# scalable-matrix/CRP-SpMM

Measured on AMD Instinct MI355X. Metric: SpMM GFLOP/s (pwtk stand-in n=256, fp64), higher is better.
Workload: dtype f64

## Files before the change

### crp-spmm_amd/_lib.py

```python
import ctypes as C
import os

_HERE = os.path.dirname(os.path.abspath(__file__))
LIB_PATH = os.environ.get("CRPSPMM_LIB_PATH") or os.path.join(_HERE, "lib", "libcrpspmm_hip.so")


class CrpLibraryError(RuntimeError):
    pass


class CrpHipError(RuntimeError):
    pass


c_int_p = C.POINTER(C.c_int)
c_dbl_p = C.POINTER(C.c_double)
c_ll_p = C.POINTER(C.c_longlong)
c_sz_p = C.POINTER(C.c_size_t)
c_u64_p = C.POINTER(C.c_uint64)

A2A_FN = C.CFUNCTYPE(None, C.c_void_p, c_int_p, c_int_p, C.c_int)
A2AV_FN = C.CFUNCTYPE(None, C.c_void_p, c_int_p, c_int_p, c_int_p, c_int_p, c_int_p, c_int_p)
AGV_FN = C.CFUNCTYPE(None, C.c_void_p, C.c_void_p, C.c_size_t, C.c_void_p, c_sz_p, c_sz_p)
BARRIER_FN = C.CFUNCTYPE(None, C.c_void_p)
# ... 45 lines not shown


class CrpspmmView(C.Structure):
    _fields_ = [(k, C.c_int) for k in ("np_glb", "rank_glb", "np_row", "np_col", "rank_row", "rank_col", "glb_m", "glb_n",
                                       "glb_k", "loc_A_srow", "loc_A_erow", "loc_A_nrow", "loc_A_nnz", "loc_A_nnz_s",
                                       "rd_B_srow", "rd_B_erow", "loc_B_scol", "loc_B_ecol", "loc_B_ncol", "loc_B_srow",
                                       "loc_B_erow", "loc_B_nrow", "a2a_B_finegrain")] + \
               [("loc_A_rowptr", c_int_p), ("loc_A_colidx", c_int_p), ("loc_A_val", c_dbl_p), ("red_B", c_dbl_p),
                ("loc_C", c_dbl_p), ("n_exec", C.c_int)] + \
               [(k, C.c_double) for k in ("t_init", "t_exec", "t_rd_A", "t_agv_A", "t_rd_B", "t_a2a_B", "t_spmm", "t_rd_C",
                                          "t_exec_nr")] + \
               [(k, C.c_size_t) for k in ("nelem_A_rd", "nelem_A_agv", "nelem_B_rd", "nelem_B_a2av", "nelem_B_a2av_min")]


_V = C.c_void_p
_I = C.c_int
_LL = C.c_longlong

SIGNATURES = {
    "crp_hip_version": (C.c_char_p, []),
    "crp_hip_device_count": (_I, [c_int_p]),
    "crp_hip_set_device": (_I, [_I]),
    "crp_hip_get_device": (_I, [c_int_p]),
    "crp_hip_device_info": (_I, [_I, C.c_char_p, c_int_p, c_sz_p]),
    "crp_hip_device_bus_id": (_I, [C.c_char_p, C.c_size_t]),
    "crp_dev_malloc": (_I, [C.POINTER(_V), C.c_size_t]),
    "crp_dev_free": (_I, [_V]),
    "crp_dev_memset": (_I, [_V, _I, C.c_size_t, _V]),
    "crp_dev_memcpy": (_I, [_V, _V, C.c_size_t, _I, _V]),
    "crp_dev_memcpy2d": (_I, [_V, C.c_size_t, _V, C.c_size_t, C.c_size_t, C.c_size_t, _I, _V]),
    "crp_host_malloc": (_I, [C.POINTER(_V), C.c_size_t]),
    "crp_host_free": (_I, [_V]),
    "crp_dev_ptr_is_device": (_I, [_V, c_int_p]),
    "crp_stream_create": (_I, [C.POINTER(_V)]),
    "crp_stream_destroy": (_I, [_V]),
    "crp_stream_sync": (_I, [_V]),
    "crp_event_create": (_I, [C.POINTER(_V)]),
    "crp_event_destroy": (_I, [_V]),
    "crp_event_record": (_I, [_V, _V]),
    "crp_event_sync": (_I, [_V]),
    "crp_stream_wait_event": (_I, [_V, _V]),
    "crp_event_elapsed_ms": (_I, [_V, _V, C.POINTER(C.c_float)]),
    "crp_csr_dev_create": (_I, [_I, _I, c_int_p, c_int_p, c_dbl_p, C.POINTER(_V)]),
    "crp_csr_dev_create_dv": (_I, [_I, _I, c_int_p, c_int_p, c_dbl_p, _V, c_int_p, C.POINTER(_V)]),
    "crp_csr_dev_destroy": (_I, [C.POINTER(_V)]),
    "crp_csr_dev_update_values": (_I, [_V, _V, _V]),
    "crp_csr_dev_set_rowmap": (_I, [_V, c_int_p, _I]),
    "crp_csr_dev_nrow": (_I, [_V]),
    "crp_csr_dev_nnz": (_LL, [_V]),
    "crp_csr_dev_bytes": (_LL, [_V]),
    "crp_csr_dev_row_part_comm_size": (_I, [_V, _I, c_int_p, c_int_p, c_int_p, c_int_p]),
    "crp_csr_dev_auto_variant": (_I, [_V]),
    "crp_csr_dev_reordered": (_I, [_V]),
    "crp_csr_dev_resolved_variant": (_I, [_V, _I]),
    "crp_csr_dev_last_variant": (_I, [_V]),
    "crp_csr_dev_lattice": (_I, [_V]),
    "crp_csr_dev_team2_compact": (_I, [_V]),
    "crp_panel_format_host": (_I, [_I, c_int_p, c_int_p, c_dbl_p, _I, c_int_p, C.POINTER(c_int_p), C.POINTER(c_int_p),
                                   C.POINTER(C.POINTER(C.c_uint)), C.POINTER(c_dbl_p), C.POINTER(_LL),
                                   C.POINTER(c_int_p), c_int_p]),
    "crp_team_format_host": (_I, [_I, c_int_p, c_int_p, c_dbl_p, c_int_p, c_int_p, C.POINTER(c_int_p), C.POINTER(c_int_p),
                                  C.POINTER(c_int_p), C.POINTER(C.POINTER(C.c_uint)), C.POINTER(c_int_p)]),
    "crp_probe_copy": (_I, [C.c_longlong, _V, _V, _I, _V, _V]),
    "crp_probe_stamp": (_I, [_V, _V]),
    "crp_stream_create_cu_mask": (_I, [C.POINTER(_V), _I, C.POINTER(C.c_uint)]),
    "crp_team2_format_host_grid": (_I, [C.POINTER(c_int_p), c_int_p]),
# ... 171 lines not shown
```

### crp-spmm_amd/csrc/dispatch.cpp

```cpp
#include "dispatch.h"
#include "locality.h"
#include "panel_format.h"

namespace crp {

constexpr int TEAM2_MIN_N = 96;
constexpr int TEAM2_HALF_FULL_LO = 61, TEAM2_HALF_FULL_HI = 64;
constexpr int TEAM2_MIN_N_NOLATTICE = 48;
constexpr int TEAM2_MIN_N_DENSE = 33;
constexpr int TEAM2_MIN_N_SPARSE = 33;
constexpr int TEAM2_MIN_N_F32 = 32, TEAM2_MIN_N_F32_SPARSE = 65;

FormatOrder format_order(int nrow, int ncol, const int *rowptr, const int *colidx, bool two_source)
{
    FormatOrder o;
    const long long nnz = rowptr[nrow];
    if (!(nnz > 0 && nrow >= 2048 && nrow == ncol && !two_source && nnz <= 200000000LL))
        return o;
    const int mode = knobs().reorder;
    std::vector<int> perm;
    if (mode == 0 || !locality_reorder(nrow, ncol, rowptr, colidx, 8, &perm)) return o;
    o.f_rowptr.assign((size_t) nrow + 1, 0);
    for (int i = 0; i < nrow; i++) o.f_rowptr[(size_t) i + 1] = o.f_rowptr[(size_t) i] + (rowptr[perm[(size_t) i] + 1] - rowptr[perm[(size_t) i]]);
    o.f_colidx.resize((size_t) nnz);
    o.f_nz.resize((size_t) nnz);
    for (int i = 0; i < nrow; i++)
    {
        const int r = perm[(size_t) i];
        int q = o.f_rowptr[(size_t) i];
        for (int pz = rowptr[r]; pz < rowptr[r + 1]; pz++, q++)
        {
            o.f_colidx[(size_t) q] = colidx[pz];
// ... 56 lines not shown
}
template bool team2_applicable<double>(const Operand &);
template bool team2_applicable<float>(const Operand &);

static bool team2_width(const MatrixTraits &t, int n)
{
    return n >= t.team2_min_n || (t.team2_min_n == TEAM2_MIN_N && n >= TEAM2_HALF_FULL_LO && n <= TEAM2_HALF_FULL_HI);
}

int resolve_f64(const MatrixTraits &t, const Operand &op, int variant, bool team2r_refused, const Knobs &k)
{
    const int n = op.n;
    const bool rows = t.nnz > 0 && t.nrow >= 8;
    int v = (variant == 0) ? t.auto_variant : variant;
    if (variant == 0 && t.team2_pays && team2_width(t, n) && team2_applicable<double>(op)) v = 5;
    const int panel_or_csr = panel_applicable(op) && t.nnz > 0 ? 3 : 1;
    if (v == 5) return team2_applicable<double>(op) && rows ? 5 : panel_or_csr;
    const int G = n <= 32 ? 4 : 2;
    const bool team2r_auto = k.team2r >= 0 ? k.team2r != 0 : (t.panels_sparse && !team2r_refused);
    if (variant == 0 && t.team2_pays && team2r_auto && n <= 64 && rows && team2r_applicable(op, G)) v = team2r_refused ? 3 : 7;
    if (v == 7) return team2r_applicable(op, G) && rows ? 7 : panel_or_csr;
    if (v >= 2 && (!panel_applicable(op) || t.nnz == 0)) v = 1;
    return v;
}

int resolve_f32(const MatrixTraits &t, const Operand &op, int variant)
{
    const int min_n = t.panels_sparse ? TEAM2_MIN_N_F32_SPARSE : TEAM2_MIN_N_F32;
    const bool team = (variant == 5 || (variant == 0 && t.team2_pays && op.n >= min_n)) && t.nnz > 0 && t.nrow >= 8 &&
                      team2_applicable<float>(op);
    return team ? 5 : 1;
}

bool team2_compact(double fill, bool for_f32)
{
    return knobs().team2_compact >= 0 ? knobs().team2_compact != 0 : (fill < 0.4 || !for_f32);
}

}
```

### crp-spmm_amd/csrc/dispatch.h

```cpp
#pragma once
#include <stdint.h>
#include <vector>
#include "knobs.h"

namespace crp {

struct FormatOrder
{
    std::vector<int>      perm, f_rowptr, f_colidx;
    std::vector<uint32_t> f_nz;
};
FormatOrder format_order(int nrow, int ncol, const int *rowptr, const int *colidx, bool two_source);

struct MatrixTraits
{
    int       nrow = 0;
    long long nnz = 0;
    int       auto_variant = 1;
    bool      team2_pays = false;
    int       team2_min_n = 96;
    bool      panels_sparse = false;
};
MatrixTraits matrix_traits(int nrow, const int *rowptr, const int *colidx);

struct Operand
{
    int       n = 0;
    long long ldB0 = 0, ldB1 = 0, ldC = 0;
    bool      has_b1 = false;
    bool      aligned16 = true;
};
bool panel_applicable(const Operand &op);
bool team2r_applicable(const Operand &op, int G);
template <typename T> bool team2_applicable(const Operand &op);

int resolve_f64(const MatrixTraits &t, const Operand &op, int variant, bool team2r_refused, const Knobs &k);
int resolve_f32(const MatrixTraits &t, const Operand &op, int variant);

bool team2_compact(double fill, bool for_f32);

}
```

### crp-spmm_amd/csrc/hip_api.hip

```cpp
#include <hip/hip_runtime.h>
#include <stdio.h>
#include <stdlib.h>
#include <string.h>
#include <new>
#include <memory>
#include <algorithm>
#include <array>
#include <vector>
#include "crpspmm_hip.h"
#include "kernels.h"
#include "panel_format.h"
#include "dispatch.h"
#include "locality.h"
#include "knobs.h"

template <typename T> struct DevBuf
{
    T *p = nullptr;
    DevBuf() = default;
    DevBuf(DevBuf &&o) noexcept : p(o.p) { o.p = nullptr; }
    DevBuf &operator=(DevBuf &&o) noexcept { std::swap(p, o.p); return *this; }
    ~DevBuf() { reset(); }
    void reset() { if (p) (void) hipFree(p); p = nullptr; }
    hipError_t alloc(size_t bytes) { reset(); return hipMalloc((void **) &p, bytes); }
// ... 363 lines not shown
int crp_dev_memcpy(void *dst, const void *src, size_t bytes, int kind, void *stream)
{
    if (bytes == 0) return 0;
    if (kind < 0 || kind > 2) return -1;
    CRP_TRY(hipMemcpyAsync(dst, src, bytes, k_copy_kinds[kind], (hipStream_t) stream));
    return 0;
}

int crp_dev_memcpy2d(void *dst, size_t dpitch, const void *src, size_t spitch, size_t width_bytes, size_t height,
                     int kind, void *stream)
{
    if (width_bytes == 0 || height == 0) return 0;
    if (kind < 0 || kind > 2) return -1;
    CRP_TRY(hipMemcpy2DAsync(dst, dpitch, src, spitch, width_bytes, height, k_copy_kinds[kind], (hipStream_t) stream));
    return 0;
}

int crp_host_malloc(void **ptr, size_t bytes)
{
    if (ptr == NULL) return -1;
    *ptr = NULL;
    if (bytes == 0) return 0;
    CRP_TRY(hipHostMalloc(ptr, bytes, hipHostMallocDefault));
    return 0;
}

int crp_host_free(void *ptr)
{
    if (ptr == NULL) return 0;
    CRP_TRY(hipHostFree(ptr));
    return 0;
}

int crp_dev_ptr_is_device(const void *ptr, int *is_dev)
{
    if (is_dev == NULL) return -1;
    *is_dev = 0;
    if (ptr == NULL) return 0;
    hipPointerAttribute_t attr;
    hipError_t e = hipPointerGetAttributes(&attr, ptr);
    if (e != hipSuccess)
    {
        (void) hipGetLastError();
        return 0;
    }
    *is_dev = (attr.type == hipMemoryTypeDevice) ? 1 : 0;
    return 0;
}

int crp_stream_create(void **stream)
{
    if (stream == NULL) return -1;
    hipStream_t s;
    CRP_TRY(hipStreamCreateWithFlags(&s, hipStreamNonBlocking));
    *stream = (void *) s;
    return 0;
}
int crp_stream_create_cu_mask(void **stream, int nwords, const unsigned *mask32)
{
    if (stream == NULL || nwords <= 0 || mask32 == NULL) return -1;
    hipStream_t s;
    CRP_TRY(hipExtStreamCreateWithCUMask(&s, (uint32_t) nwords, mask32));
    *stream = (void *) s;
    return 0;
}
int crp_probe_copy(long long bytes, const void *src, void *dst, int blocks, unsigned long long *stamps, void *stream)
// ... 314 lines not shown
    if (C == NULL || (B0 == NULL && B1 == NULL && A->nnz > 0)) return -1;
    if (ldC < n || (B0 && ldB0 < n) || (B1 && ldB1 < n)) return -4;
    const hipStream_t s = (hipStream_t) stream;
    if (A->val32 == nullptr)
    {
        CRP_TRY(A->val32.alloc(sizeof(float) * (size_t) (A->nnz > 0 ? A->nnz : 1)));
        CRP_TRY(crp::convert_f64_f32(A->nnz, A->val, A->val32, s));
    }
    crp::SpmmArgsF32 a;
    a.nrow = A->nrow; a.n = n; a.rowptr = A->rowptr; a.colidx = A->colidx; a.val = A->val32;
    a.B0 = B0; a.ldB0 = ldB0; a.B1 = B1; a.ldB1 = ldB1; a.C = C; a.ldC = ldC; a.rowmap = A->rowmap;
    A->last_variant = crp::resolve_f32(A->traits, operand_of(n, B0, ldB0, B1, ldB1, C, ldC), variant);
    if (A->last_variant == 1) return (int) crp::spmm_rm_f32_rowgroup(a, s);
    const int rc = ensure_team2(A, s, true);
    if (rc != 0) return rc;
    Team2Dev &d = A->team2;
    if (d.tval32 == nullptr)
    {
        CRP_TRY(d.tval32.alloc(sizeof(float) * ((size_t) d.value_entries + 1024)));
        CRP_TRY(hipMemsetAsync(d.tval32, 0, sizeof(float) * ((size_t) d.value_entries + 1024), s));
        CRP_TRY(crp::convert_f64_f32(d.value_entries, d.tval, d.tval32, s));
    }
    if (A->rowmap_fmt != nullptr) a.rowmap = A->rowmap_fmt;
    crp::Team2Args t;
    team2_args(d, &t);
    return (int) crp::spmm_rm_f32_team2(t, a, s);
}

int crp_csr_dev_auto_variant(crp_csr_dev_p A) { return A ? A->traits.auto_variant : -1; }
int crp_csr_dev_reordered(crp_csr_dev_p A) { return A ? (A->ord.perm.empty() ? 0 : 1) : -1; }
int crp_csr_dev_resolved_variant(crp_csr_dev_p A, int n)
{
    return A ? crp::resolve_f64(A->traits, operand_of(n, nullptr, n, nullptr, 0, nullptr, n), 0, A->team2r_refused, crp::knobs()) : -1;
}
int crp_csr_dev_last_variant(crp_csr_dev_p A) { return A ? A->last_variant : -1; }
int crp_csr_dev_lattice(crp_csr_dev_p A) { return A ? ((A->team2.built && A->team2.lattice) ? 1 : 0) : -1; }
int crp_csr_dev_team2_compact(crp_csr_dev_p A) { return (A && A->team2.built) ? (A->team2.compact ? 1 : 0) : -1; }

int crp_panel_format_host(int nrow, const int *rowptr, const int *colidx, const double *val, int R, int *npanel,
                          int **pptr, int **pcol, unsigned **pmask4, double **pval, long long *real_entries,
                          int **porder, int *norder)
{
    if (nrow < 0 || rowptr == NULL || (R != 4 && R != 8) || !npanel || !pptr || !pcol || !pmask4 || !pval) return -1;
    crp::PanelHost h;
    crp::build_panels(nrow, rowptr, colidx, val, R, &h);
    *npanel = h.npanel;
    *pptr = dup(h.pptr);
    *pcol = dup(h.pcol);
    *pmask4 = dup(h.pmask4);
    *pval = dup(h.pval);
    if (real_entries) *real_entries = h.real_entries;
    if (norder) *norder = (int) h.porder.size();
    if (porder) *porder = dup(h.porder);
    return 0;
}

int crp_team_format_host(int nrow, const int *rowptr, const int *colidx, const double *val, int *nteam, int *lattice,
                         int **tpanel, int **tptr, int **tcol, unsigned **tmask, int **torder)
{
    if (nrow < 0 || rowptr == NULL || !nteam || !tpanel || !tptr || !tcol || !tmask || !torder) return -1;
    crp::PanelHost h;
    crp::build_panels(nrow, rowptr, colidx, val, 8, &h, false);
    crp::TeamHost th;
    crp::build_teams(h, nrow, rowptr, colidx, &th);
    *nteam = th.nteam;
    if (lattice) *lattice = th.lattice ? 1 : 0;
// ... 167 lines not shown
```

### crp-spmm_amd/csrc/kernels.h

```cpp
#pragma once
#include <hip/hip_runtime.h>
#include <stdint.h>

namespace crp {

struct SpmmArgs
{
    int nrow;
    int n;
    const int    *rowptr;
    const int    *colidx;
    const double *val;
    const double *B0;
    int64_t       ldB0;
    const double *B1;
    int64_t       ldB1;
    double       *C;
    int64_t       ldC;
    const int    *rowmap;
};

struct SpmmArgsF32
{
    int nrow;
// ... 48 lines not shown
    int G;
    int nteam;
    int ngrid;
    const int      *tgrid;
    const int      *tpanel;
    const int      *tinfo;
    const uint32_t *trec;
    const long long *tvoff;
    const double   *tval;
    uint32_t       *tent;
};

bool spmm_narrow_applicable(const PanelArgs &p, const SpmmArgs &a);
hipError_t spmm_rm_f64_narrow(const PanelArgs &p, const SpmmArgs &a, hipStream_t s);

hipError_t spmm_rm_f64_rowgroup(const SpmmArgs &a, hipStream_t s);
hipError_t spmm_cm_f64(const SpmmArgs &a, hipStream_t s);
hipError_t spmm_rm_f64_panel(const PanelArgs &p, const SpmmArgs &a, hipStream_t s);

hipError_t spmm_rm_f64_team2r(const Team2NArgs &t, const SpmmArgs &a, hipStream_t s);
hipError_t team2r_fill_rows(const Team2NArgs &t, const SpmmArgs &a, hipStream_t s);

hipError_t spmm_rm_f64_team2(const Team2Args &t, const SpmmArgs &a, hipStream_t s);
hipError_t spmm_rm_f32_team2(const Team2Args &t, const SpmmArgsF32 &a, hipStream_t s);

hipError_t spmm_rm_f32_rowgroup(const SpmmArgsF32 &a, hipStream_t s);

hipError_t gather_rows_f64(int layout, int nidx, int n, const int *ridx, const double *src, int64_t lds,
                           double *dst, int64_t ldd, hipStream_t s);
hipError_t scatter_rows_f64(int layout, int nidx, int n, const int *ridx, const double *src, int64_t lds,
                            double *dst, int64_t ldd, hipStream_t s);
hipError_t scatter_vals_f64(int64_t n, const uint32_t *map, const double *src, double *dst, hipStream_t s);
hipError_t convert_f64_f32(int64_t n, const double *src, float *dst, hipStream_t s);
hipError_t transpose_f64(int nrow, int ncol, const double *src, int64_t lds, double *dst, int64_t ldd,
                         hipStream_t s);
hipError_t gather_rows_f32(int layout, int nidx, int n, const int *ridx, const float *src, int64_t lds,
                           float *dst, int64_t ldd, hipStream_t s);
hipError_t scatter_rows_f32(int layout, int nidx, int n, const int *ridx, const float *src, int64_t lds,
                            float *dst, int64_t ldd, hipStream_t s);
hipError_t transpose_f32(int nrow, int ncol, const float *src, int64_t lds, float *dst, int64_t ldd, hipStream_t s);
hipError_t row_part_comm_size(int nrow, int ncol, const int *rowptr, const int *colidx, int nblk, const int *rblk_dev, const int *xd_dev,
                              unsigned *bits, int *comm_dev, int *bad_dev, hipStream_t s);
hipError_t probe_copy(int64_t bytes, const void *src, void *dst, int blocks, unsigned long long *stamps, hipStream_t s);
hipError_t probe_stamp(unsigned long long *out, hipStream_t s);

}
```

### crp-spmm_amd/csrc/knobs.cpp

```cpp
#include <stdlib.h>
#include <string.h>
#include <algorithm>
#include "knobs.h"

namespace crp {

static int env_int(const char *name, int dflt)
{
    const char *v = getenv(name);
    return (v != NULL && *v != 0) ? atoi(v) : dflt;
}

static bool env_is(const char *name, const char *what)
{
    const char *v = getenv(name);
    return v != NULL && strcmp(v, what) == 0;
}

static Knobs read_knobs()
{
    Knobs k;
    k.timing = env_int("CRPSPMM_TIMING", 0) != 0;
    k.num_threads = std::max(0, env_int("CRPSPMM_NUM_THREADS", env_int("OMP_NUM_THREADS", 0)));
    k.sync_release = getenv("CRPSPMM_SYNC_RELEASE") != NULL;
    k.spmm_variant = env_int("CRPSPMM_SPMM_VARIANT", 0);
    k.reorder = env_int("CRPSPMM_REORDER", -1);
    k.panel_order = env_int("CRPSPMM_PANEL_ORDER", -1);
    k.team2_compact = env_int("CRPSPMM_TEAM2_COMPACT", -1);
    k.team2r = env_int("CRPSPMM_TEAM2R", -1);
    k.t2_latorder = env_int("CRPSPMM_T2_LATORDER", 1) != 0;
    k.overlap = env_int("CRPSPMM_OVERLAP", 1);
    k.exchange_host = env_is("CRPSPMM_EXCHANGE", "host");
    k.replicate_host = env_is("CRPSPMM_REPLICATE", "host");
    {
        const char *v = getenv("CRPSPMM_RCCL_TIMEOUT");
        const double t = v ? atof(v) : 120.0;
        k.rccl_timeout = t > 0.0 ? t : 120.0;
    }
    k.rccl_blocking = env_int("CRPSPMM_RCCL_BLOCKING", 0) != 0;
    k.engine_a_static = env_int("CRPSPMM_ENGINE_A_STATIC", -1);
    return k;
}

const Knobs &knobs()
{
    static const bool live = env_int("CRPSPMM_KNOBS_LIVE", 0) != 0;
    static Knobs k = read_knobs();
    if (live) k = read_knobs();
    return k;
}

}
```

### crp-spmm_amd/csrc/knobs.h

```cpp
#pragma once

namespace crp {

struct Knobs
{
    bool   timing;
    int    num_threads;
    bool   sync_release;
    int    spmm_variant;
    int    reorder;
    int    panel_order;
    int    team2_compact;
    int    team2r;
    bool   t2_latorder;
    int    overlap;
    bool   exchange_host;
    bool   replicate_host;
    double rccl_timeout;
    bool   rccl_blocking;
    int    engine_a_static;
};

const Knobs &knobs();

}
```

### crp-spmm_amd/csrc/row_kernels.hip

```cpp
#include <hip/hip_runtime.h>
#include <algorithm>
#include <stdint.h>
#include "kernels.h"

namespace crp {

typedef double d2 __attribute__((ext_vector_type(2)));

static inline int grid_for(int64_t work)
{
    int64_t blocks = (work + 255) / 256;
    if (blocks > 2048) blocks = 2048;
    if (blocks < 1) blocks = 1;
    return (int) blocks;
}

template <int VW, bool GATHER>
__global__ __launch_bounds__(256) void move_rows_rm_kernel(
    const int64_t nidx, const int cpr , const int *__restrict__ ridx,
    const double *__restrict__ src, const int64_t lds, double *__restrict__ dst, const int64_t ldd)
{
    const int64_t total = nidx * (int64_t) cpr;
    for (int64_t t = (int64_t) blockIdx.x * 256 + threadIdx.x; t < total; t += (int64_t) gridDim.x * 256)
    {
// ... 224 lines not shown
{
    if (nrow <= 0 || ncol <= 0) return hipSuccess;
    dim3 grid((nrow + 31) / 32, (ncol + 31) / 32);
    hipLaunchKernelGGL(transpose_f32_kernel, grid, dim3(256), 0, s, nrow, ncol, src, lds, dst, ldd);
    return hipGetLastError();
}

__global__ __launch_bounds__(256) void scatter_vals_kernel(const int64_t n, const uint32_t *__restrict__ map,
                                                           const double *__restrict__ src, double *__restrict__ dst)
{
    for (int64_t i = (int64_t) blockIdx.x * 256 + threadIdx.x; i < n; i += (int64_t) gridDim.x * 256) dst[map[i]] = src[i];
}

hipError_t scatter_vals_f64(int64_t n, const uint32_t *map, const double *src, double *dst, hipStream_t s)
{
    if (n <= 0) return hipSuccess;
    hipLaunchKernelGGL(scatter_vals_kernel, dim3(grid_for(n)), dim3(256), 0, s, n, map, src, dst);
    return hipGetLastError();
}

__global__ void convert_f64_f32_kernel(const int64_t n, const double *__restrict__ src, float *__restrict__ dst)
{
    for (int64_t i = (int64_t) blockIdx.x * blockDim.x + threadIdx.x; i < n; i += (int64_t) gridDim.x * blockDim.x) dst[i] = (float) src[i];
}

hipError_t convert_f64_f32(int64_t n, const double *src, float *dst, hipStream_t s)
{
    if (n <= 0) return hipSuccess;
    const int blocks = (int) ((n + 255) / 256 < 4096 ? (n + 255) / 256 : 4096);
    hipLaunchKernelGGL(convert_f64_f32_kernel, dim3(blocks), dim3(256), 0, s, n, src, dst);
    return hipGetLastError();
}

__global__ __launch_bounds__(256) void probe_copy_kernel(const int64_t n16, const uint4 *__restrict__ src, uint4 *__restrict__ dst,
                                                          unsigned long long *__restrict__ stamps)
{
    if (threadIdx.x == 0) atomicMin(&stamps[0], (unsigned long long) wall_clock64());
    for (int64_t i = (int64_t) blockIdx.x * 256 + threadIdx.x; i < n16; i += (int64_t) gridDim.x * 256) dst[i] = src[i];
    __syncthreads();
    if (threadIdx.x == 0) atomicMax(&stamps[1], (unsigned long long) wall_clock64());
}

__global__ void probe_stamp_kernel(unsigned long long *__restrict__ out) { *out = (unsigned long long) wall_clock64(); }

hipError_t probe_copy(int64_t bytes, const void *src, void *dst, int blocks, unsigned long long *stamps, hipStream_t s)
{
    if (bytes <= 0 || blocks <= 0) return hipErrorInvalidValue;
    hipLaunchKernelGGL(probe_copy_kernel, dim3(blocks), dim3(256), 0, s, bytes / 16, (const uint4 *) src, (uint4 *) dst, stamps);
    return hipGetLastError();
}

hipError_t probe_stamp(unsigned long long *out, hipStream_t s)
{
    hipLaunchKernelGGL(probe_stamp_kernel, dim3(1), dim3(1), 0, s, out);
    return hipGetLastError();
}

__global__ void comm_mark_kernel(const int nrow, const int *__restrict__ rowptr, const int *__restrict__ colidx, const int nblk,
                                 const int *__restrict__ rblk, const long long words, unsigned *__restrict__ bits, int *__restrict__ bad)
{
    const int lane = threadIdx.x & 63;
    const long long wave0 = ((long long) blockIdx.x * blockDim.x + threadIdx.x) >> 6, nwave = ((long long) gridDim.x * blockDim.x) >> 6;
    for (long long r = wave0; r < nrow; r += nwave)
    {
        int lo = 0, hi = nblk;
        while (hi - lo > 1)
// ... 57 lines not shown
```

### crp-spmm_amd/csrc/rp_engine.cpp

```cpp
#include <limits.h>
#include <stdio.h>
#include <stdlib.h>
#include <string.h>
#include <vector>
#include "crp_engine.h"
#include "crpspmm_hip.h"
#include "utils.h"
#include "par.h"
#include <algorithm>

struct crp_rp_spmm
{
    int nproc = 1, my_rank = 0, glb_n = 0, A_nrow = 0, rB_nrow = 0;
    int rB_self_src_offset = 0, rB_self_dst_offset = 0, rB_self_nrow = 0;
    int rB_p2p = 1, rB_reidx = 1;
    std::vector<int>       A_rowptr, A_colidx;
    std::vector<double>    A_val;
    std::vector<int>       rB_self_src_ridxs, rB_sridxs, rB_rridxs;
    std::vector<long long> rB_scnts, rB_sdispls, rB_rcnts, rB_rdispls;
    size_t rB_recv_size = 0;
    int    n_exec = 0;
    double t_init = 0, t_pack = 0, t_a2a = 0, t_unpack = 0, t_spmm = 0, t_exec = 0;
    bool vals_from_device = false;
    double t_a2a_host = 0;
    crp_comm_t *comm = nullptr;

    bool plan_only = false;
    int  timing = 1, variant = 0;
    int  variant_f32 = 0;
    int  loc_B_nrow = 0;
    long long n_send_rows = 0, n_recv_rows = 0, n_needed_rows = 0;
    std::vector<int> dev_colidx_host;
    crp_csr_dev_p A_dev = nullptr;
    crp_csr_dev_p A_int = nullptr, A_bnd = nullptr;
    std::vector<long long> int_src, bnd_src;
    std::vector<double>    split_vals;
    void *xstream = nullptr, *ev_packed = nullptr, *ev_landed = nullptr;
    int    *sridxs_dev = nullptr;
    double *sendbuf_dev = nullptr, *recvbuf_dev = nullptr;
    bool   x32_ready = false;
    float *sendbuf32_dev = nullptr, *recvbuf32_dev = nullptr;
    std::vector<long long> x32_scnts, x32_sdispls, x32_rcnts, x32_rdispls;
    void   *stream = nullptr;
    double *B_stage = nullptr, *C_stage = nullptr, *B_rm = nullptr, *C_rm = nullptr;
    size_t  B_stage_sz = 0, C_stage_sz = 0, B_rm_sz = 0, C_rm_sz = 0;
    void *ev_exec = nullptr;
    bool  exec_pending = false;
    const void *last_B = nullptr, *last_C = nullptr;
    int last_B_dev = 0, last_C_dev = 0;
};

#define HIP_OK(call)                                                              \
    do {                                                                          \
        int rc__ = (call);                                                        \
        ASSERT_PRINTF(rc__ == 0, "%s failed with code %d\n", #call, rc__);        \
    } while (0)

static void grow(double **buf, size_t *cur, size_t need_elems)
{
    if (need_elems <= *cur) return;
    if (*buf) HIP_OK(crp_dev_free(*buf));
    void *p = NULL;
    HIP_OK(crp_dev_malloc(&p, need_elems * sizeof(double)));
    *buf = (double *) p;
    *cur = need_elems;
}


static void build_plan(crp_rp_spmm *e, int A_nrow, const int *A_rowptr, const int *A_colidx,
                       const double *A_val, const int *B_row_displs, int glb_n, crp_comm_t *comm)
{
    const int P = comm->nproc, me = comm->rank;
    e->nproc = P;
    e->my_rank = me;
    e->glb_n = glb_n;
    e->A_nrow = A_nrow;
    e->comm = comm;
    GET_ENV_INT_VAR(e->rB_p2p, "RP_SPMM_P2P", "rB_p2p", 1, 0, 1, me == 0);
    GET_ENV_INT_VAR(e->rB_reidx, "RP_SPMM_REIDX", "rB_reidx", 1, 0, 1, me == 0);

    const int    base = A_rowptr[0];
    const size_t nnz  = (size_t) ((long long) A_rowptr[A_nrow] - (long long) base);
    const int    glb_k = B_row_displs[P];
    const int    lo = B_row_displs[me], hi = B_row_displs[me + 1];
    e->loc_B_nrow = hi - lo;

    std::vector<unsigned char> flag((size_t) glb_k + 1, 0);
    int cmin = INT_MAX, cmax = -1;
    for (size_t p = 0; p < nnz; p++)
// ... 196 lines not shown
{
    (void) A_srow;
    rp_init_common(A_nrow, A_rowptr, A_colidx, A_val, B_row_displs, glb_n, comm, rp_spmm, false, A_val_dev);
}

int crp_rp_spmm_values_from_device(crp_rp_spmm_p e) { return (e && e->vals_from_device) ? 1 : 0; }

void crp_rp_spmm_init_plan_only(int A_srow, int A_nrow, const int *A_rowptr, const int *A_colidx,
                                const double *A_val, const int *B_row_displs, int glb_n, crp_comm_t *comm,
                                crp_rp_spmm_p *rp_spmm)
{
    (void) A_srow;
    rp_init_common(A_nrow, A_rowptr, A_colidx, A_val, B_row_displs, glb_n, comm, rp_spmm, true);
}

void crp_rp_spmm_free(crp_rp_spmm_p *rp_spmm)
{
    if (rp_spmm == NULL || *rp_spmm == NULL) return;
    crp_rp_spmm *e = *rp_spmm;
    if (!e->plan_only)
    {
        crp_csr_dev_destroy(&e->A_dev);
        crp_csr_dev_destroy(&e->A_int);
        crp_csr_dev_destroy(&e->A_bnd);
        if (e->xstream) crp_stream_destroy(e->xstream);
        if (e->ev_packed) crp_event_destroy(e->ev_packed);
        if (e->ev_landed) crp_event_destroy(e->ev_landed);
        crp_dev_free(e->sridxs_dev);
        crp_dev_free(e->sendbuf_dev);
        crp_dev_free(e->recvbuf_dev);
        crp_dev_free(e->sendbuf32_dev);
        crp_dev_free(e->recvbuf32_dev);
        if (e->ev_exec) crp_event_destroy(e->ev_exec);
        crp_dev_free(e->B_stage);
        crp_dev_free(e->C_stage);
        crp_dev_free(e->B_rm);
        crp_dev_free(e->C_rm);
        crp_stream_destroy(e->stream);
    }
    delete e;
    *rp_spmm = NULL;
}

}

static long long ld32_of(int n) { return ((long long) n + 3) / 4 * 4; }

template <class T> static T *grow_as(double **buf, size_t *cur, size_t need_elems)
{
    grow(buf, cur, (need_elems * sizeof(T) + sizeof(double) - 1) / sizeof(double));
    return (T *) *buf;
}

struct Xchg
{
    void *send, *recv;
    long long ld;
    const long long *sc, *sd, *rc, *rd;
};

static Xchg exchange_of(crp_rp_spmm *e, const double *)
{
    return Xchg{e->sendbuf_dev, e->recvbuf_dev, (long long) e->glb_n, e->rB_scnts.data(), e->rB_sdispls.data(),
                e->rB_rcnts.data(), e->rB_rdispls.data()};
}

// ... 24 lines not shown
        HIP_OK(crp_stream_sync(NULL));
        e->x32_ready = true;
    }
    return Xchg{e->sendbuf32_dev, e->recvbuf32_dev, ld, e->x32_scnts.data(), e->x32_sdispls.data(), e->x32_rcnts.data(),
                e->x32_rdispls.data()};
}

static int gather(int nidx, int n, const int *ridx, const double *src, long long lds, double *dst, long long ldd, void *s)
{
    return crp_gather_rows_f64(0, nidx, n, ridx, src, lds, dst, ldd, s);
}
static int gather(int nidx, int n, const int *ridx, const float *src, long long lds, float *dst, long long ldd, void *s)
{
    return crp_gather_rows_f32(0, nidx, n, ridx, src, lds, dst, ldd, s);
}
static int transpose(int nrow, int ncol, const double *src, long long lds, double *dst, long long ldd, void *s)
{
    return crp_transpose_f64(nrow, ncol, src, lds, dst, ldd, s);
}
static int transpose(int nrow, int ncol, const float *src, long long lds, float *dst, long long ldd, void *s)
{
    return crp_transpose_f32(nrow, ncol, src, lds, dst, ldd, s);
}
static int spmm(crp_rp_spmm *e, crp_csr_dev_p A, int n, const double *B0, long long ldB0, const double *B1, long long ldB1,
                double *C, long long ldC, void *s)
{
    return crp_spmm_csr_f64(A, 0, n, B0, ldB0, B1, ldB1, C, ldC, e->variant, s);
}
static int spmm(crp_rp_spmm *e, crp_csr_dev_p A, int n, const float *B0, long long ldB0, const float *B1, long long ldB1,
                float *C, long long ldC, void *s)
{
    return crp_spmm_csr_f32(A, n, B0, ldB0, B1, ldB1, C, ldC, e->variant_f32, s);
}

template <class T>
static void exec_impl(crp_rp_spmm *e, int BC_layout, const T *B, long long ldB, T *C, long long ldC, void *stream_)
{
    if (e == NULL) return;
    ASSERT_PRINTF(!e->plan_only, "rp_spmm_exec on a plan-only engine (no device state)\n");
    ASSERT_PRINTF(BC_layout == 0 || BC_layout == 1, "BC_layout must be 0 or 1\n");
    const double t_begin = get_wtime_sec();
    void *s = stream_;
    const int n = e->glb_n, kb = e->loc_B_nrow, m = e->A_nrow;
    const bool timing = e->timing != 0;
    double t0, t1;

    int B_on_dev = 0, C_on_dev = 0;
    if (B == e->last_B && B != NULL) B_on_dev = e->last_B_dev;
    else
    {
        HIP_OK(crp_dev_ptr_is_device(B, &B_on_dev));
        e->last_B = B;
        e->last_B_dev = B_on_dev;
    }
    if (C == e->last_C && C != NULL) C_on_dev = e->last_C_dev;
    else
    {
        HIP_OK(crp_dev_ptr_is_device(C, &C_on_dev));
        e->last_C = C;
        e->last_C_dev = C_on_dev;
    }

    const Xchg x = exchange_of(e, B);
    const T *Bd = B;
    long long ldBd = ldB;
    if (!B_on_dev && kb > 0 && n > 0)
    {
        const size_t elems = (BC_layout == 0) ? (size_t) kb * (size_t) ldB : (size_t) n * (size_t) ldB;
        T *stage = grow_as<T>(&e->B_stage, &e->B_stage_sz, elems);
        const size_t used = (BC_layout == 0) ? ((size_t) (kb - 1) * (size_t) ldB + (size_t) n)
                                             : ((size_t) (n - 1) * (size_t) ldB + (size_t) kb);
        HIP_OK(crp_dev_memcpy(stage, B, used * sizeof(T), 0, s));
        Bd = stage;
    }
    if (BC_layout == 1 && kb > 0 && n > 0)
    {
        T *rm = grow_as<T>(&e->B_rm, &e->B_rm_sz, (size_t) kb * (size_t) n);
        HIP_OK(transpose(n, kb, Bd, ldB, rm, n, s));
        Bd = rm;
        ldBd = n;
    }
    T *Cd = C;
    long long ldCd = ldC;
    if (BC_layout == 1)
    {
        Cd = grow_as<T>(&e->C_rm, &e->C_rm_sz, (size_t) m * (size_t) n);
        ldCd = n;
    }
    else if (!C_on_dev && m > 0 && n > 0)
    {
        Cd = grow_as<T>(&e->C_stage, &e->C_stage_sz, (size_t) m * (size_t) ldC);
    }

// ... 298 lines not shown
```

### include/crpspmm_hip.h

```cpp
#ifndef CRPSPMM_HIP_H
#define CRPSPMM_HIP_H

#include <stddef.h>
#include <stdint.h>

#ifdef __cplusplus
extern "C" {
#endif

#define CRP_LAYOUT_ROW_MAJOR 0
#define CRP_LAYOUT_COL_MAJOR 1

typedef struct crp_csr_dev *crp_csr_dev_p;

int crp_hip_device_count(int *count);
int crp_hip_set_device(int dev);
int crp_hip_get_device(int *dev);
int crp_hip_device_info(int dev, char *name, int *cu_count, size_t *hbm_bytes);

int crp_hip_device_bus_id(char *out, size_t len);

int crp_dev_malloc(void **ptr, size_t bytes);
int crp_dev_free(void *ptr);
int crp_dev_memset(void *ptr, int value, size_t bytes, void *stream);
int crp_dev_memcpy(void *dst, const void *src, size_t bytes, int kind, void *stream);
int crp_dev_memcpy2d(void *dst, size_t dpitch, const void *src, size_t spitch, size_t width_bytes,
                     size_t height, int kind, void *stream);
int crp_host_malloc(void **ptr, size_t bytes);
int crp_host_free(void *ptr);
int crp_dev_ptr_is_device(const void *ptr, int *is_dev);

int crp_stream_create(void **stream);
int crp_stream_destroy(void *stream);
int crp_stream_sync(void *stream);
int crp_event_create(void **event);
int crp_event_destroy(void *event);
int crp_event_record(void *event, void *stream);
int crp_event_sync(void *event);
int crp_stream_wait_event(void *stream, void *event);
int crp_event_elapsed_ms(void *start, void *stop, float *ms);

int crp_csr_dev_create(int nrow, int ncol, const int *rowptr, const int *colidx,
                       const double *val, crp_csr_dev_p *out);
int crp_csr_dev_create_dv(int nrow, int ncol, const int *rowptr, const int *colidx, const double *val_host,
                          const double *val_dev, const int *src_start, crp_csr_dev_p *out);
int crp_csr_dev_destroy(crp_csr_dev_p *A);
int crp_csr_dev_update_values(crp_csr_dev_p A, const double *val, void *stream);
int crp_csr_dev_set_rowmap(crp_csr_dev_p A, const int *rowmap, int c_nrow);
int crp_csr_dev_nrow(crp_csr_dev_p A);
long long crp_csr_dev_nnz(crp_csr_dev_p A);
long long crp_csr_dev_bytes(crp_csr_dev_p A);
int crp_csr_dev_row_part_comm_size(crp_csr_dev_p A, int nblk, const int *rblk_ptr, const int *x_displs, int *comm_sizes,
                                   int *total_size);

int crp_spmm_csr_f32(crp_csr_dev_p A, int n, const float *B0, long long ldB0, const float *B1, long long ldB1, float *C,
                     long long ldC, int variant, void *stream);

int crp_csr_dev_auto_variant(crp_csr_dev_p A);
int crp_csr_dev_reordered(crp_csr_dev_p A);
int crp_csr_dev_resolved_variant(crp_csr_dev_p A, int n);
int crp_csr_dev_last_variant(crp_csr_dev_p A);
int crp_csr_dev_lattice(crp_csr_dev_p A);
int crp_csr_dev_team2_compact(crp_csr_dev_p A);
int crp_panel_format_host(int nrow, const int *rowptr, const int *colidx, const double *val, int R,
                          int *npanel, int **pptr, int **pcol, unsigned **pmask4, double **pval,
                          long long *real_entries, int **porder, int *norder);

int crp_team_format_host(int nrow, const int *rowptr, const int *colidx, const double *val, int *nteam, int *lattice,
                         int **tpanel, int **tptr, int **tcol, unsigned **tmask, int **torder);

int crp_team2_format_host(int nrow, const int *rowptr, const int *colidx, const double *val, int *nteam, int *lattice,
                          int **tpanel, int **tinfo, int **tpro, unsigned **trec, long long *nrecwords,
                          long long **tvoff, double **tval, long long *nvalent, int **torder, unsigned **vmap);
int crp_team2_format_host_grid(int **tgrid, int *ngrid);
int crp_team2_format_host_compact(void);

int crp_team2r_format_host(int nrow, const int *rowptr, const int *colidx, const double *val, int G, int *nteam, int *lattice, int **tpanel,
                           int **tinfo, unsigned **trec, long long *nrecwords, long long **tvoff, double **tval, long long *nwords,
                           int **tgrid, int *ngrid, unsigned **vmap, long long *stats, unsigned **tent);

int crp_locality_order_host(int nrow, int ncol, const int *rowptr, const int *colidx, int nparts, int *perm, double *info);
int crp_spmm_plan_host(int nrow, int ncol, const int *rowptr, const int *colidx, int nwidth, const int *widths, int variant, int f32,
                       int shape, int *resolved, int *info);

int crp_spmm_csr_f64(crp_csr_dev_p A, int layout, int n,
                     const double *B0, long long ldB0,
                     const double *B1, long long ldB1,
                     double *C, long long ldC, int variant, void *stream);
const char *crp_spmm_variant_name(int variant);
int crp_spmm_variant_count(void);

int crp_gather_rows_f64(int layout, int nidx, int n, const int *ridx,
                        const double *src, long long lds,
// ... 26 lines not shown
```

Baseline: 19910.

## Pipeline host-resident B/C transfers with SpMM by splitting columns into tiles

Measured after the change: 19490. -2.1%, worse.

```diff
diff --git a/crp-spmm_amd/_lib.py b/crp-spmm_amd/_lib.py
--- a/crp-spmm_amd/_lib.py
+++ b/crp-spmm_amd/_lib.py
@@ -101,6 +101,12 @@
     "crp_host_malloc": (_I, [C.POINTER(_V), C.c_size_t]),
     "crp_host_free": (_I, [_V]),
     "crp_dev_ptr_is_device": (_I, [_V, c_int_p]),
+    "crp_dev_copy_rows": (_I, [_V, C.c_size_t, _V, C.c_size_t, C.c_size_t, C.c_size_t, _V]),
+    "crp_host_register": (_I, [_V, C.c_size_t, c_int_p]),
+    "crp_host_unregister": (_I, [_V]),
+    "crp_spmm_resolve_f64": (_I, [_V, _I, _V, _LL, _V, _LL, _V, _LL, _I]),
+    "crp_spmm_resolve_f32": (_I, [_V, _I, _V, _LL, _V, _LL, _V, _LL, _I]),
+    "crp_host_tiles": (_I, [_I, _I, _I, c_int_p]),
     "crp_stream_create": (_I, [C.POINTER(_V)]),
     "crp_stream_destroy": (_I, [_V]),
     "crp_stream_sync": (_I, [_V]),
diff --git a/crp-spmm_amd/csrc/dispatch.cpp b/crp-spmm_amd/csrc/dispatch.cpp
--- a/crp-spmm_amd/csrc/dispatch.cpp
+++ b/crp-spmm_amd/csrc/dispatch.cpp
@@ -1,3 +1,4 @@
+#include <algorithm>
 #include "dispatch.h"
 #include "locality.h"
 #include "panel_format.h"
@@ -120,6 +121,18 @@
     return team ? 5 : 1;
 }
 
+std::vector<int> host_tiles(int n, int elem_size, int variant)
+{
+    std::vector<int> edges{0, n > 0 ? n : 0};
+    if (variant != 5 || n <= 0 || (elem_size != 8 && elem_size != 4)) return edges;
+    const int vw = 16 / elem_size, min_w = 512 / elem_size;
+    const int T = std::min(HOST_TILES_MAX, n / min_w);
+    if (T < 2) return edges;
+    edges.assign((size_t) T + 1, n);
+    for (int t = 0; t < T; t++) edges[(size_t) t] = (int) ((long long) t * n / T / vw * vw);
+    return edges;
+}
+
 bool team2_compact(double fill, bool for_f32)
 {
     return knobs().team2_compact >= 0 ? knobs().team2_compact != 0 : (fill < 0.4 || !for_f32);
diff --git a/crp-spmm_amd/csrc/dispatch.h b/crp-spmm_amd/csrc/dispatch.h
--- a/crp-spmm_amd/csrc/dispatch.h
+++ b/crp-spmm_amd/csrc/dispatch.h
@@ -37,6 +37,9 @@
 int resolve_f64(const MatrixTraits &t, const Operand &op, int variant, bool team2r_refused, const Knobs &k);
 int resolve_f32(const MatrixTraits &t, const Operand &op, int variant);
 
+constexpr int HOST_TILES_MAX = 4;
+std::vector<int> host_tiles(int n, int elem_size, int variant);
+
 bool team2_compact(double fill, bool for_f32);
 
 }
diff --git a/crp-spmm_amd/csrc/hip_api.hip b/crp-spmm_amd/csrc/hip_api.hip
--- a/crp-spmm_amd/csrc/hip_api.hip
+++ b/crp-spmm_amd/csrc/hip_api.hip
@@ -419,6 +419,50 @@
     return 0;
 }
 
+int crp_dev_copy_rows(void *dst, size_t dpitch, const void *src, size_t spitch, size_t width_bytes, size_t height, void *stream)
+{
+    CRP_TRY(crp::copy_rows_16b((int64_t) height, (int64_t) width_bytes, src, (int64_t) spitch, dst, (int64_t) dpitch, (hipStream_t) stream));
+    return 0;
+}
+
+int crp_host_register(const void *ptr, size_t bytes, int *state)
+{
+    if (state == NULL) return -1;
+    *state = 0;
+    if (ptr == NULL || bytes == 0) return 0;
+    hipPointerAttribute_t attr;
+    hipError_t e = hipPointerGetAttributes(&attr, ptr);
+    if (e != hipSuccess) (void) hipGetLastError();
+    else if (attr.type == hipMemoryTypeHost) *state = 2;
+    else if (attr.type != hipMemoryTypeUnregistered) return 0;
+    if (*state == 0)
+    {
+        e = hipHostRegister(const_cast<void *>(ptr), bytes, hipHostRegisterDefault);
+        if (e != hipSuccess)
+        {
+            (void) hipGetLastError();
+            return 0;
+        }
+        *state = 1;
+    }
+    void *dptr = NULL;
+    e = hipHostGetDevicePointer(&dptr, const_cast<void *>(ptr), 0);
+    if (e != hipSuccess || dptr != ptr)
+    {
+        (void) hipGetLastError();
+        if (*state == 1) (void) hipHostUnregister(const_cast<void *>(ptr));
+        *state = 0;
+    }
+    return 0;
+}
+
+int crp_host_unregister(const void *ptr)
+{
+    if (ptr == NULL) return 0;
+    CRP_TRY(hipHostUnregister(const_cast<void *>(ptr)));
+    return 0;
+}
+
 int crp_dev_ptr_is_device(const void *ptr, int *is_dev)
 {
     if (is_dev == NULL) return -1;
@@ -799,6 +843,25 @@
 int crp_csr_dev_resolved_variant(crp_csr_dev_p A, int n)
 {
     return A ? crp::resolve_f64(A->traits, operand_of(n, nullptr, n, nullptr, 0, nullptr, n), 0, A->team2r_refused, crp::knobs()) : -1;
+}
+int crp_spmm_resolve_f64(crp_csr_dev_p A, int n, const double *B0, long long ldB0, const double *B1, long long ldB1, const double *C, long long ldC,
+                         int variant)
+{
+    if (A == NULL || !variant_valid(variant, false)) return -1;
+    return crp::resolve_f64(A->traits, operand_of(n, B0, ldB0, B1, ldB1, C, ldC), variant, A->team2r_refused, crp::knobs());
+}
+int crp_spmm_resolve_f32(crp_csr_dev_p A, int n, const float *B0, long long ldB0, const float *B1, long long ldB1, const float *C, long long ldC,
+                         int variant)
+{
+    if (A == NULL || !variant_valid(variant, true)) return -1;
+    return crp::resolve_f32(A->traits, operand_of(n, B0, ldB0, B1, ldB1, C, ldC), variant);
+}
+int crp_host_tiles(int n, int elem_size, int variant, int *edges)
+{
+    if (edges == NULL) return -1;
+    const std::vector<int> e = crp::host_tiles(n, elem_size, variant);
+    for (size_t t = 0; t < e.size(); t++) edges[t] = e[t];
+    return (int) e.size() - 1;
 }
 int crp_csr_dev_last_variant(crp_csr_dev_p A) { return A ? A->last_variant : -1; }
 int crp_csr_dev_lattice(crp_csr_dev_p A) { return A ? ((A->team2.built && A->team2.lattice) ? 1 : 0) : -1; }
diff --git a/crp-spmm_amd/csrc/kernels.h b/crp-spmm_amd/csrc/kernels.h
--- a/crp-spmm_amd/csrc/kernels.h
+++ b/crp-spmm_amd/csrc/kernels.h
@@ -104,6 +104,7 @@
                             double *dst, int64_t ldd, hipStream_t s);
 hipError_t scatter_vals_f64(int64_t n, const uint32_t *map, const double *src, double *dst, hipStream_t s);
 hipError_t convert_f64_f32(int64_t n, const double *src, float *dst, hipStream_t s);
+hipError_t copy_rows_16b(int64_t nrow, int64_t width_bytes, const void *src, int64_t spitch_bytes, void *dst, int64_t dpitch_bytes, hipStream_t s);
 hipError_t transpose_f64(int nrow, int ncol, const double *src, int64_t lds, double *dst, int64_t ldd,
                          hipStream_t s);
 hipError_t gather_rows_f32(int layout, int nidx, int n, const int *ridx, const float *src, int64_t lds,
diff --git a/crp-spmm_amd/csrc/knobs.cpp b/crp-spmm_amd/csrc/knobs.cpp
--- a/crp-spmm_amd/csrc/knobs.cpp
+++ b/crp-spmm_amd/csrc/knobs.cpp
@@ -39,6 +39,7 @@
     }
     k.rccl_blocking = env_int("CRPSPMM_RCCL_BLOCKING", 0) != 0;
     k.engine_a_static = env_int("CRPSPMM_ENGINE_A_STATIC", -1);
+    k.host_pipeline = env_int("CRPSPMM_HOST_PIPELINE", 1) != 0;
     return k;
 }
 
diff --git a/crp-spmm_amd/csrc/knobs.h b/crp-spmm_amd/csrc/knobs.h
--- a/crp-spmm_amd/csrc/knobs.h
+++ b/crp-spmm_amd/csrc/knobs.h
@@ -19,6 +19,7 @@
     double rccl_timeout;
     bool   rccl_blocking;
     int    engine_a_static;
+    bool   host_pipeline;
 };
 
 const Knobs &knobs();
diff --git a/crp-spmm_amd/csrc/row_kernels.hip b/crp-spmm_amd/csrc/row_kernels.hip
--- a/crp-spmm_amd/csrc/row_kernels.hip
+++ b/crp-spmm_amd/csrc/row_kernels.hip
@@ -280,6 +280,28 @@
     return hipGetLastError();
 }
 
+__global__ __launch_bounds__(256) void copy_rows_16b_kernel(const int64_t nrow, const int w16, const uint4 *__restrict__ src, const int64_t spitch16,
+                                                             uint4 *__restrict__ dst, const int64_t dpitch16)
+{
+    const int64_t total = nrow * w16;
+    for (int64_t i = (int64_t) blockIdx.x * 256 + threadIdx.x; i < total; i += (int64_t) gridDim.x * 256)
+    {
+        const int64_t r = i / w16;
+        const int c = (int) (i - r * w16);
+        dst[r * dpitch16 + c] = src[r * spitch16 + c];
+    }
+}
+
+hipError_t copy_rows_16b(int64_t nrow, int64_t width_bytes, const void *src, int64_t spitch_bytes, void *dst, int64_t dpitch_bytes, hipStream_t s)
+{
+    if (nrow <= 0 || width_bytes <= 0) return hipSuccess;
+    if ((width_bytes | spitch_bytes | dpitch_bytes | (int64_t) (uintptr_t) src | (int64_t) (uintptr_t) dst) & 15) return hipErrorInvalidValue;
+    if (width_bytes > spitch_bytes || width_bytes > dpitch_bytes || width_bytes / 16 > INT32_MAX) return hipErrorInvalidValue;
+    hipLaunchKernelGGL(copy_rows_16b_kernel, dim3(256), dim3(256), 0, s, nrow, (int) (width_bytes / 16), (const uint4 *) src, spitch_bytes / 16,
+                       (uint4 *) dst, dpitch_bytes / 16);
+    return hipGetLastError();
+}
+
 __global__ __launch_bounds__(256) void probe_copy_kernel(const int64_t n16, const uint4 *__restrict__ src, uint4 *__restrict__ dst,
                                                           unsigned long long *__restrict__ stamps)
 {
diff --git a/crp-spmm_amd/csrc/rp_engine.cpp b/crp-spmm_amd/csrc/rp_engine.cpp
--- a/crp-spmm_amd/csrc/rp_engine.cpp
+++ b/crp-spmm_amd/csrc/rp_engine.cpp
@@ -7,7 +7,15 @@
 #include "crpspmm_hip.h"
 #include "utils.h"
 #include "par.h"
+#include "dispatch.h"
 #include <algorithm>
+
+struct HostReg
+{
+    const void *ptr = nullptr;
+    size_t bytes = 0;
+    int state = 0;
+};
 
 struct crp_rp_spmm
 {
@@ -48,6 +56,9 @@
     bool  exec_pending = false;
     const void *last_B = nullptr, *last_C = nullptr;
     int last_B_dev = 0, last_C_dev = 0;
+    HostReg reg_B, reg_C;
+    void *up_stream = nullptr, *down_stream = nullptr, *ev_begin = nullptr, *ev_down = nullptr;
+    void *ev_up[crp::HOST_TILES_MAX] = {}, *ev_k0[crp::HOST_TILES_MAX] = {}, *ev_k1[crp::HOST_TILES_MAX] = {};
 };
 
 #define HIP_OK(call)                                                              \
@@ -55,6 +66,26 @@
         int rc__ = (call);                                                        \
         ASSERT_PRINTF(rc__ == 0, "%s failed with code %d\n", #call, rc__);        \
     } while (0)
+
+static void unpin(HostReg *r)
+{
+    if (r->state == 1) (void) crp_host_unregister(r->ptr);
+    *r = HostReg();
+}
+
+static bool pin(HostReg *r, const void *p, size_t bytes)
+{
+    if (r->ptr != p || r->bytes != bytes)
+    {
+        unpin(r);
+        int st = 0;
+        HIP_OK(crp_host_register(p, bytes, &st));
+        r->ptr = p;
+        r->bytes = bytes;
+        r->state = st;
+    }
+    return r->state != 0;
+}
 
 static void grow(double **buf, size_t *cur, size_t need_elems)
 {
@@ -317,6 +348,18 @@
         crp_dev_free(e->sendbuf32_dev);
         crp_dev_free(e->recvbuf32_dev);
         if (e->ev_exec) crp_event_destroy(e->ev_exec);
+        unpin(&e->reg_B);
+        unpin(&e->reg_C);
+        if (e->up_stream) crp_stream_destroy(e->up_stream);
+        if (e->down_stream) crp_stream_destroy(e->down_stream);
+        if (e->ev_begin) crp_event_destroy(e->ev_begin);
+        if (e->ev_down) crp_event_destroy(e->ev_down);
+        for (int t = 0; t < crp::HOST_TILES_MAX; t++)
+        {
+            if (e->ev_up[t]) crp_event_destroy(e->ev_up[t]);
+            if (e->ev_k0[t]) crp_event_destroy(e->ev_k0[t]);
+            if (e->ev_k1[t]) crp_event_destroy(e->ev_k1[t]);
+        }
         crp_dev_free(e->B_stage);
         crp_dev_free(e->C_stage);
         crp_dev_free(e->B_rm);
@@ -407,6 +450,99 @@
 {
     return crp_spmm_csr_f32(A, n, B0, ldB0, B1, ldB1, C, ldC, e->variant_f32, s);
 }
+static int spmm_as(int variant, crp_csr_dev_p A, int n, const double *B, long long ldB, double *C, long long ldC, void *s)
+{
+    return crp_spmm_csr_f64(A, 0, n, B, ldB, NULL, 0, C, ldC, variant, s);
+}
+static int spmm_as(int variant, crp_csr_dev_p A, int n, const float *B, long long ldB, float *C, long long ldC, void *s)
+{
+    return crp_spmm_csr_f32(A, n, B, ldB, NULL, 0, C, ldC, variant, s);
+}
+static int resolved(crp_rp_spmm *e, int n, const double *B, long long ldB, const double *C, long long ldC)
+{
+    return crp_spmm_resolve_f64(e->A_dev, n, B, ldB, NULL, 0, C, ldC, e->variant);
+}
+static int resolved(crp_rp_spmm *e, int n, const float *B, long long ldB, const float *C, long long ldC)
+{
+    return crp_spmm_resolve_f32(e->A_dev, n, B, ldB, NULL, 0, C, ldC, e->variant_f32);
+}
+
+template <class T>
+static bool exec_host_tiles(crp_rp_spmm *e, int layout, const T *B, long long ldB, bool B_on_dev, T *C, long long ldC, bool C_on_dev, void *s)
+{
+    const int n = e->glb_n, kb = e->loc_B_nrow, m = e->A_nrow;
+    if (!crp::knobs().host_pipeline || e->nproc != 1 || e->A_dev == nullptr || (B_on_dev && C_on_dev) || n <= 0 || kb <= 0 || m <= 0)
+        return false;
+    const bool cm = layout == 1;
+    const size_t B_rows = cm ? (size_t) n : (size_t) kb, B_len = cm ? (size_t) kb : (size_t) n;
+    const size_t C_rows = cm ? (size_t) n : (size_t) m, C_len = cm ? (size_t) m : (size_t) n;
+    const T *Bs = B_on_dev ? B : grow_as<T>(&e->B_stage, &e->B_stage_sz, B_rows * (size_t) ldB);
+    T *Cs = C_on_dev ? C : grow_as<T>(&e->C_stage, &e->C_stage_sz, C_rows * (size_t) ldC);
+    const T *Bd = cm ? grow_as<T>(&e->B_rm, &e->B_rm_sz, (size_t) kb * (size_t) n) : Bs;
+    T *Cd = cm ? grow_as<T>(&e->C_rm, &e->C_rm_sz, (size_t) m * (size_t) n) : Cs;
+    const long long ldBd = cm ? n : ldB, ldCd = cm ? n : ldC;
+    const int variant = resolved(e, n, Bd, ldBd, Cd, ldCd);
+    const std::vector<int> edge = crp::host_tiles(n, (int) sizeof(T), variant);
+    const int ntile = (int) edge.size() - 1;
+    if (ntile < 2) return false;
+    if (!cm && !C_on_dev && (uintptr_t) C % 16 != 0) return false;
+    if (!B_on_dev && !pin(&e->reg_B, B, ((B_rows - 1) * (size_t) ldB + B_len) * sizeof(T))) return false;
+    if (!C_on_dev && !pin(&e->reg_C, C, ((C_rows - 1) * (size_t) ldC + C_len) * sizeof(T))) return false;
+    if (e->up_stream == nullptr)
+    {
+        HIP_OK(crp_stream_create(&e->up_stream));
+        HIP_OK(crp_stream_create(&e->down_stream));
+        HIP_OK(crp_event_create(&e->ev_begin));
+        HIP_OK(crp_event_create(&e->ev_down));
+        for (int t = 0; t < crp::HOST_TILES_MAX; t++)
+        {
+            HIP_OK(crp_event_create(&e->ev_up[t]));
+            HIP_OK(crp_event_create(&e->ev_k0[t]));
+            HIP_OK(crp_event_create(&e->ev_k1[t]));
+        }
+    }
+    const bool timing = e->timing != 0;
+    const size_t pB = (size_t) ldB * sizeof(T), pC = (size_t) ldC * sizeof(T);
+    HIP_OK(crp_event_record(e->ev_begin, s));
+    HIP_OK(crp_stream_wait_event(e->up_stream, e->ev_begin));
+    HIP_OK(crp_stream_wait_event(e->down_stream, e->ev_begin));
+    for (int t = 0; t < ntile; t++)
+    {
+        const int c0 = edge[(size_t) t], w = edge[(size_t) t + 1] - c0;
+        if (!B_on_dev)
+        {
+            if (cm) HIP_OK(crp_dev_memcpy2d((T *) Bs + (size_t) c0 * ldB, pB, B + (size_t) c0 * ldB, pB, (size_t) kb * sizeof(T), (size_t) w, 0, e->up_stream));
+            else HIP_OK(crp_dev_memcpy2d((T *) Bs + c0, pB, B + c0, pB, (size_t) w * sizeof(T), (size_t) kb, 0, e->up_stream));
+            HIP_OK(crp_event_record(e->ev_up[t], e->up_stream));
+            HIP_OK(crp_stream_wait_event(s, e->ev_up[t]));
+        }
+        if (timing) HIP_OK(crp_event_record(e->ev_k0[t], s));
+        if (cm) HIP_OK(transpose(w, kb, Bs + (size_t) c0 * ldB, ldB, (T *) Bd + c0, n, s));
+        HIP_OK(spmm_as(variant, e->A_dev, w, Bd + c0, ldBd, Cd + c0, ldCd, s));
+        if (cm) HIP_OK(transpose(m, w, Cd + c0, n, Cs + (size_t) c0 * ldC, ldC, s));
+        if (timing || !C_on_dev) HIP_OK(crp_event_record(e->ev_k1[t], s));
+        if (!C_on_dev)
+        {
+            HIP_OK(crp_stream_wait_event(e->down_stream, e->ev_k1[t]));
+            if (cm) HIP_OK(crp_dev_memcpy2d(C + (size_t) c0 * ldC, pC, Cs + (size_t) c0 * ldC, pC, (size_t) m * sizeof(T), (size_t) w, 1, e->down_stream));
+            else HIP_OK(crp_dev_copy_rows(C + c0, pC, Cs + c0, pC, (size_t) w * sizeof(T), (size_t) m, e->down_stream));
+        }
+    }
+    if (!C_on_dev)
+    {
+        HIP_OK(crp_event_record(e->ev_down, e->down_stream));
+        HIP_OK(crp_stream_wait_event(s, e->ev_down));
+    }
+    HIP_OK(crp_stream_sync(s));
+    if (timing)
+        for (int t = 0; t < ntile; t++)
+        {
+            float ms = 0.f;
+            HIP_OK(crp_event_elapsed_ms(e->ev_k0[t], e->ev_k1[t], &ms));
+            e->t_spmm += 1e-3 * (double) ms;
+        }
+    return true;
+}
 
 template <class T>
 static void exec_impl(crp_rp_spmm *e, int BC_layout, const T *B, long long ldB, T *C, long long ldC, void *stream_)
@@ -434,6 +570,13 @@
         HIP_OK(crp_dev_ptr_is_device(C, &C_on_dev));
         e->last_C = C;
         e->last_C_dev = C_on_dev;
+    }
+
+    if (exec_host_tiles(e, BC_layout, B, ldB, B_on_dev != 0, C, ldC, C_on_dev != 0, s))
+    {
+        e->t_exec += get_wtime_sec() - t_begin;
+        e->n_exec++;
+        return;
     }
 
     const Xchg x = exchange_of(e, B);
diff --git a/include/crpspmm_hip.h b/include/crpspmm_hip.h
--- a/include/crpspmm_hip.h
+++ b/include/crpspmm_hip.h
@@ -29,6 +29,10 @@
 int crp_host_malloc(void **ptr, size_t bytes);
 int crp_host_free(void *ptr);
 int crp_dev_ptr_is_device(const void *ptr, int *is_dev);
+int crp_dev_copy_rows(void *dst, size_t dpitch, const void *src, size_t spitch, size_t width_bytes, size_t height,
+                      void *stream);
+int crp_host_register(const void *ptr, size_t bytes, int *state);
+int crp_host_unregister(const void *ptr);
 
 int crp_stream_create(void **stream);
 int crp_stream_destroy(void *stream);
@@ -59,6 +63,11 @@
 int crp_csr_dev_auto_variant(crp_csr_dev_p A);
 int crp_csr_dev_reordered(crp_csr_dev_p A);
 int crp_csr_dev_resolved_variant(crp_csr_dev_p A, int n);
+int crp_spmm_resolve_f64(crp_csr_dev_p A, int n, const double *B0, long long ldB0, const double *B1, long long ldB1,
+                         const double *C, long long ldC, int variant);
+int crp_spmm_resolve_f32(crp_csr_dev_p A, int n, const float *B0, long long ldB0, const float *B1, long long ldB1,
+                         const float *C, long long ldC, int variant);
+int crp_host_tiles(int n, int elem_size, int variant, int *edges);
 int crp_csr_dev_last_variant(crp_csr_dev_p A);
 int crp_csr_dev_lattice(crp_csr_dev_p A);
 int crp_csr_dev_team2_compact(crp_csr_dev_p A);
```
